# aidagroup/quad-periodic-mpc

Hardware: AMD Instinct MI355X
Metric: QP solves/sec (N=10, 13-state, 12-force) at batch=65536; 1/2/4/8 GPU (higher is better)
Workload: dtype f32

## Files before the change

quad-periodic-mpc_amd/build.py:

```python
from __future__ import annotations

import os
import re
import subprocess
from concurrent.futures import ThreadPoolExecutor

PKG = os.path.dirname(os.path.abspath(__file__))
ROOT = os.path.dirname(PKG)
CSRC = os.path.join(PKG, "csrc")
LIB = os.path.join(PKG, "libcmpc_hip.so")
OBJ = os.path.join(ROOT, "build", "obj")
SOURCES = ["cmpc_tail.hip", "cmpc_wide_w256.hip", "cmpc_wide_w192.hip", "cmpc_class1.hip", "cmpc_wide_w80.hip", "cmpc_wide_w96.hip",
           "cmpc_wide_w120.hip", "cmpc_wide_w128.hip", "cmpc_wide_w144.hip", "cmpc_wide_w80p.hip",
           "cmpc_wide_w96p.hip", "cmpc_wide_w120p.hip", "cmpc_wide_w128p.hip", "cmpc_wide_w80r.hip",
           "cmpc_wide_w96r.hip", "cmpc_wide_w120r.hip", "cmpc_wide_w80pr.hip", "cmpc_wide_w96pr.hip",
           "cmpc_wide_w120pr.hip", "cmpc_wide_w96prd.hip", "cmpc_wide_w120prd.hip", "cmpc_wide_w96rd.hip", "cmpc_wide_w120rd.hip", "cmpc_condense.hip", "cmpc_launch.hip", "cmpc_estimator.hip", "cmpc_assemble.hip",
           "cmpc_admm.hip", "cmpc_quadprog.hip", "cmpc_evaluate.hip", "cmpc_abi.cpp"]
ARCH = os.environ.get("CMPC_OFFLOAD_ARCH", "gfx950")
FLAGS = ["-O3", "-std=c++17", "-fPIC", "-Wall", "-Wno-unused-result", "-fno-slp-vectorize", "-ffp-contract=on"]


def _deps(path: str, seen=None) -> set:
    seen = set() if seen is None else seen
    path = os.path.normpath(path)
    if path in seen or not os.path.exists(path):
        return seen
    seen.add(path)
    for inc in re.findall(r'#include\s+"([^"]+)"', open(path).read()):
        _deps(os.path.join(os.path.dirname(path), inc), seen)
    return seen


def _obj(src: str, defines: tuple) -> str:
    tag = ("_" + "_".join(d.replace("=", "-") for d in defines)) if defines else ""
    return os.path.join(OBJ, f"{src}{tag}.o")


def _stale(target: str, deps) -> bool:
    if not os.path.exists(target):
        return True
    t = os.path.getmtime(target)
    return any(os.path.getmtime(d) > t for d in deps)


def build(force: bool = False, verbose: bool = False, out: str | None = None,
          defines: tuple = ()) -> str:
    lib = out or LIB
    hipcc = os.environ.get("HIPCC", "/opt/rocm/bin/hipcc")
    os.makedirs(OBJ, exist_ok=True)

    def compile_one(src: str) -> str:
        path = os.path.join(CSRC, src)
        obj = _obj(src, defines)
        if not force and not _stale(obj, _deps(path)):
            return obj
        cmd = [hipcc, f"--offload-arch={ARCH}", *FLAGS, *[f"-D{d}" for d in defines], "-c", path,
               "-o", obj + ".tmp"]
        if src.endswith(".cpp"):
            cmd[1:1] = ["-x", "hip"]
        if verbose:
            print(" ".join(cmd), flush=True)
        subprocess.run(cmd, check=True)
        os.replace(obj + ".tmp", obj)
        return obj

    jobs = max(1, min(len(SOURCES), int(os.environ.get("MAX_JOBS", os.cpu_count() or 1))))
    with ThreadPoolExecutor(jobs) as ex:
        objs = list(ex.map(compile_one, SOURCES))
    if not force and not _stale(lib, objs):
        return lib
    tmp = lib + ".tmp"
    subprocess.run([hipcc, f"--offload-arch={ARCH}", "-shared", "-fPIC", "-o", tmp] + objs,
                   check=True)
    os.replace(tmp, lib)
    if out is None:
        build_tools(lib)
        build_multi(lib)
    return lib


MULTI_LIB = os.path.join(PKG, "libcmpc_multi.so")


def build_multi(lib: str = LIB) -> str:
    hipcc = os.environ.get("HIPCC", "/opt/rocm/bin/hipcc")
    src = os.path.join(CSRC, "cmpc_multi.cpp")
    hdrs = [os.path.join(ROOT, "include", h) for h in ("cmpc_multi.h", "cmpc_solver.h")]
    if _stale(MULTI_LIB, [src, lib] + hdrs):
        subprocess.run([hipcc, "-x", "hip", "--offload-arch=" + ARCH, "-O2", "-std=c++17", "-fPIC",
                        "-Wall", "-shared", "-o", MULTI_LIB + ".tmp", src, f"-L{PKG}", "-lcmpc_hip",
                        "-L/opt/rocm/lib", "-lrccl", "-Wl,-rpath,$ORIGIN", f"-Wl,-rpath,{PKG}",
                        "-Wl,-rpath,/opt/rocm/lib"], check=True)
        os.replace(MULTI_LIB + ".tmp", MULTI_LIB)
    exe = os.path.join(PKG, "cmpc_multi_test")
    tsrc = os.path.join(CSRC, "tools", "cmpc_multi_test.cpp")
    if _stale(exe, [tsrc, MULTI_LIB] + hdrs):
        subprocess.run([hipcc, "-x", "hip", "--offload-arch=" + ARCH, "-O2", "-std=c++17", "-o", exe + ".tmp",
                        tsrc, f"-L{PKG}", "-lcmpc_multi", "-lcmpc_hip", "-Wl,-rpath,$ORIGIN",
                        f"-Wl,-rpath,{PKG}"], check=True)
        os.replace(exe + ".tmp", exe)
    exe = os.path.join(PKG, "cmpc_multi_model_test")
    tsrc = os.path.join(CSRC, "tools", "cmpc_multi_model_test.cpp")
    if _stale(exe, [tsrc, MULTI_LIB] + hdrs):
        subprocess.run([hipcc, "-x", "hip", "--offload-arch=" + ARCH, "-O2", "-std=c++17", "-o", exe + ".tmp",
                        tsrc, f"-L{PKG}", "-lcmpc_multi", "-lcmpc_hip", "-Wl,-rpath,$ORIGIN",
                        f"-Wl,-rpath,{PKG}"], check=True)
        os.replace(exe + ".tmp", exe)
    return MULTI_LIB


def build_tools(lib: str = LIB) -> str:
    exe = os.path.join(PKG, "cmpc_abi_latency")
    src = os.path.join(CSRC, "tools", "cmpc_abi_latency.cpp")
    if not _stale(exe, [src, lib]):
        return exe
    subprocess.run(["g++", "-O2", "-std=c++17", "-o", exe + ".tmp", src, f"-L{PKG}", "-lcmpc_hip",
                    f"-Wl,-rpath,$ORIGIN", f"-Wl,-rpath,{PKG}"], check=True)
    os.replace(exe + ".tmp", exe)
    return exe


if __name__ == "__main__":
    import sys
    print(build(force="--force" in sys.argv, verbose=True))
```

quad-periodic-mpc_amd/csrc/cmpc_class1.hip:

```cpp
#include <stdlib.h>

#include "cmpc_common.h"

#ifndef CMPC_W1_WAVES_60
#define CMPC_W1_WAVES_60 4
#endif
#ifndef CMPC_W1_WAVES_PER_EU
#define CMPC_W1_WAVES_PER_EU 4
#endif
#ifndef CMPC_C1_RL
#define CMPC_C1_RL 0
#endif
#ifndef CMPC_TRIP_PRIO_AT
#define CMPC_TRIP_PRIO_AT 0
#endif
#ifndef CMPC_C1_TRIP_PRIO
#define CMPC_C1_TRIP_PRIO 2
#endif
#ifndef C1_PIPE_GRP
#define C1_PIPE_GRP 4
#endif
#ifndef CMPC_C1_CHOL2
#define CMPC_C1_CHOL2 1
#endif
#ifndef CMPC_C1_FUSEDJ
#define CMPC_C1_FUSEDJ 2
#endif
#ifndef CMPC_C1_JPIPE
#define CMPC_C1_JPIPE 1
#endif
#ifndef CMPC_C1_DOT2
#define CMPC_C1_DOT2 0
#endif
#if CMPC_C1_DOT2
#define C1_DOT dot4x2
#else
#define C1_DOT dot4
#endif
#ifndef CMPC_C1_XUNC
#define CMPC_C1_XUNC 1
#endif

#ifdef CMPC_PHASE_PROF
__device__ unsigned long long g_c1_phase[16];
#define C1_MARK(i)                              \
  do {                                          \
    const unsigned long long _n = clock64();    \
    ph[i] += _n - t_last;                       \
    t_last = _n;                                \
  } while (0)
#define C1_SUB(i)                               \
  do {                                          \
    const unsigned long long _n = clock64();    \
    ph[8 + (i)] += _n - t_sub;                  \
    t_sub = _n;                                 \
  } while (0)
#else
#define C1_MARK(i) \
  do {             \
  } while (0)
#define C1_SUB(i) \
  do {            \
  } while (0)
#endif

#ifdef CMPC_PLACE_PROF
constexpr int kPlaceMax = 65536;
__device__ unsigned int g_c1_place[4 * kPlaceMax];
#endif

namespace cmpc {
namespace {

constexpr int NL = 64;

template <int NV>
struct C1Geo {
  static constexpr int NG = NV / 4;
  static constexpr int PSZ = 4 * NG * NV - 8 * NG * (NG - 1);
  __host__ __device__ static constexpr int prow(int r) {
    return 4 * (r >> 2) * NV - 8 * (r >> 2) * ((r >> 2) - 1) + (r & 3) * (NV - 4 * (r >> 2));
  }
  __host__ __device__ static constexpr int prow0(int r) { return prow(r) - (r & ~3); }
  __host__ __device__ static constexpr int tri(int r) { return r * NV - ((r * (r + 1)) >> 1); }
  static_assert(NV * NV - ((NV * (NV + 1)) >> 1) <= 4 * NG * NV - 8 * NG * (NG - 1), "exchange fits P");
};
__device__ __forceinline__ int rcol(int j) { return (j * (j + 1)) >> 1; }
constexpr int rinv_cols(int words) {
  int q = 0;
  while ((q + 1) * (q + 2) <= words) q++;
  return q;
}

constexpr int OFF_E = 0;
constexpr int OFF_ZE = OFF_E + 16 * MAXN;
constexpr int OFF_REC = OFF_ZE + 16 * MAXN;

constexpr int C1_MAXFS = 24;

template <int NV>
struct SharedC1 {
  static_assert(NV % 4 == 0 && NV <= NL, "row width");
  static_assert(NV * (NV + 1) / 2 <= C1Geo<NV>::PSZ, "R must fit in P");
  static_assert(OFF_REC + CMPC_REC_WORDS(MAXN) <= C1Geo<NV>::PSZ, "prep scratch must fit in P");
  static_assert(3 * C1_MAXFS >= NV, "stance list");
  static_assert(NV * (NV + 1) / 2 <= C1Geo<NV>::PSZ - NL, "vbuf in P's tail");
  __device__ __forceinline__ float* vbuf() { return &P[C1Geo<NV>::PSZ - NL]; }
  static constexpr int QI = rinv_cols(C1Geo<NV>::PSZ - NL);
  static constexpr int RB = C1Geo<NV>::PSZ - NL - QI * (QI + 1) / 2;
  static_assert(QI * (QI + 1) / 2 <= RB, "R and R^-1 side by side");
  float P[C1Geo<NV>::PSZ];
  union {
    float BdtT[12][16];
    float ibuf[NL];
    struct {
      float bufA[NL], bufB[NL];
      float cs[2 * NL];
    } gi;
  } u;
  float sub[C1_MAXFS];
  int sfs[C1_MAXFS];
  int blkbase[MAXN + 2];
  unsigned char varblk[NL], varcol[NL];
  unsigned char cmask[NL];
};

__device__ __forceinline__ void lsync() {
  __builtin_amdgcn_wave_barrier();
  asm volatile("" ::: "memory");
}

__device__ __forceinline__ float fdiv(float a, float b) { return a * fast_rcp(b); }

template <int M>
__device__ __forceinline__ void pin(float (&x)[M]) {
#pragma unroll
  for (int c = 0; c < M; c++) asm volatile("" : "+v"(x[c]));
}

template <int LO, int HI, int MA>
__device__ __forceinline__ float pick_col(const float (&x)[MA], int q) {
  static_assert(0 <= LO && LO < HI && HI <= MA, "column range");
  if constexpr (HI - LO == 1) {
    float r = x[LO];
    asm volatile("" : "+v"(r));
    return r;
  } else {
    constexpr int MID = (LO + HI) / 2;
    if (q < MID) return pick_col<LO, MID>(x, q);
    return pick_col<MID, HI>(x, q);
  }
}

#ifndef CMPC_FENCE_COLS
#define CMPC_FENCE_COLS 16
#endif
#define CMPC_SWEEP_FENCE(c)                                                                  \
  do {                                                                                       \
    if (((c) & (CMPC_FENCE_COLS - 1)) == CMPC_FENCE_COLS - 4) __builtin_amdgcn_sched_barrier(0); \
  } while (0)

template <int NV>
__device__ __forceinline__ void solve_c1(const float* __restrict__ rec, const KParams& P,
                                         SharedC1<NV>& sh, float* __restrict__ fout,
                                         uint8_t* __restrict__ st_out, int32_t* __restrict__ it_out,
                                         int* __restrict__ ovf_list, int* __restrict__ ovf_count,
                                         int inst) {
  using G = C1Geo<NV>;
  const int v = threadIdx.x;
  const int N = P.N;
#ifdef CMPC_PHASE_PROF
  unsigned long long ph[16] = {0, 0, 0, 0, 0, 0, 0, 0, 0, 0, 0, 0, 0, 0, 0, 0};
  unsigned long long t_sub = 0;
  unsigned long long t_last = clock64();
#endif
  {
    const float4* src = reinterpret_cast<const float4*>(rec);
    float4* dst = reinterpret_cast<float4*>(&sh.P[OFF_REC]);
    for (int t = v; t < (P.rec_words >> 2); t += 64) dst[t] = src[t];
  }
  lsync();
  const float* srec = &sh.P[OFF_REC];
  const unsigned char* gait = reinterpret_cast<const unsigned char*>(srec + CMPC_REC_HDR + 12 * N);
  int nfs = 0;
  unsigned long long msk0 = 0ull, msk1 = 0ull;
  for (int c0 = 0; c0 < 4 * N; c0 += 64) {
    const int t = c0 + v;
    float ub = 0.f;
    bool f = false;
    if (t < 4 * N) {
      ub = (float)gait[t] * P.f_max;
      f = !(ub < 0.01f && ub > -0.01f);
    }
    const unsigned long long m = __ballot(f);
    if (c0 == 0) msk0 = m; else msk1 = m;
    const int pre = __popcll(m & ((1ull << v) - 1ull));
    if (f && nfs + pre < C1_MAXFS) {
      sh.sfs[nfs + pre] = t;
      sh.sub[nfs + pre] = ub;
    }
    nfs += __popcll(m);
  }
  const int n = 3 * nfs;
  if (n > NV) {
    if (v == 0 && ovf_list) ovf_list[atomicAdd(ovf_count, 1)] = inst;
    return;
  }
  lsync();
  {
    int kb = 0, kc = 0;
    if (v < n) {
      const int fs = sh.sfs[v / 3];
      kb = fs >> 2;
      kc = 3 * (fs & 3) + v % 3;
    }
    sh.varblk[v] = (unsigned char)kb;
    sh.varcol[v] = (unsigned char)kc;
    if (v <= N) {
      const int b0 = 4 * v, b1 = 4 * v - 64;
      const unsigned long long lo = (b0 >= 64) ? msk0 : (msk0 & ((1ull << b0) - 1ull));
      const unsigned long long hi = (b1 <= 0) ? 0ull : (msk1 & ((1ull << b1) - 1ull));
      sh.blkbase[v] = 3 * (__popcll(lo) + __popcll(hi));
    }
    for (int t = v; t < nfs; t += 64) sh.cmask[t] = 0;
  }
  Model md;
  make_model(srec, P.dt, P.mdl, md);
  make_bdt<64>(srec, md, v, sh.u.BdtT);
  CondGeo cg;
  make_cond_geo<true>(srec, md, cg);
  lsync();
  float wts[13];
#pragma unroll
  for (int j = 0; j < 12; j++) wts[j] = P.wts[j];
  wts[12] = 0.f;
  if (v < N) {
    float e[13];
    state_error(srec, md, v, srec + CMPC_REC_HDR + 12 * v, e);
#pragma unroll
    for (int j = 0; j < 13; j++) sh.P[OFF_E + 16 * v + j] = wts[j] * e[j];
  }
  lsync();
  moment_recur(&sh.P[OFF_E], &sh.P[OFF_ZE], N, v);
  lsync();
  C1_MARK(0);

  const bool real = v < n;
  float gv;
  {
    const int kv = real ? sh.varblk[v] : 0;
    const int cv = real ? sh.varcol[v] : 0;
    float b[13], u1[13], u2[13];
#pragma unroll
    for (int j = 0; j < 13; j++) b[j] = real ? sh.u.BdtT[cv][j] : 0.f;
    n1_mul(md, b, u1);
    n1_mul(md, u1, u2);
    gv = grad_from_moments(b, u1, u2, &sh.P[OFF_E + 16 * kv], &sh.P[OFF_ZE + 16 * kv]);
    gv = real ? gv : 0.f;
    lsync();
    const int myrow = G::tri(v);
    float z[13];
#pragma unroll
    for (int j = 0; j < 13; j++) z[j] = 0.f;
    for (int i = N - 1; i >= 0; i--) {
      const bool act = real && (i >= kv);
      const float k = (float)(i - kv);
      const float k2 = 0.5f * k * (k - 1.f);
      float gk[13];
      col_power(b, u1, u2, k, k2, gk);
#pragma unroll
      for (int j = 0; j < 13; j++) gk[j] = act ? gk[j] : 0.f;
      recur(md, wts, gk, z);
      asm volatile("" ::: "memory");
      const int wb = __builtin_amdgcn_readfirstlane(sh.blkbase[i]);
      step_entries(md, cg, sh.u.BdtT, step_mask(msk0, msk1, i), wb, z, [&](int w, float val) {
        if (w == v) val += P.alpha2;
        if (act && w >= v) sh.P[myrow + w] = val;
      });
    }
  }
  lsync();
  C1_MARK(1);

  float slot[NV + 1];
  {
    const int vv = (v < NV) ? v : 0;
    const int myrow = G::tri(vv);
    static_for<0, NV>([&](auto C) {
      constexpr int c = decltype(C)::value;
      const int addr = (c >= vv) ? myrow + c : G::tri(c) + vv;
      const float x = sh.P[addr];
      slot[c] = (real && c < n) ? x : ((c == v) ? 1.f : 0.f);
      if ((c & 7) == 7) __builtin_amdgcn_sched_barrier(0);
    });
    slot[NV] = gv;
  }
  lsync();

  int status = CMPC_OK;
  float my_inv = 1.f;
#if CMPC_C1_CHOL2
  float i0n = 1.f, betan = 0.f, i1n = 1.f, g0n = 0.f, g1n = 0.f;
  auto look = [&](auto JJ) {
    constexpr int j = decltype(JJ)::value, j1 = j + 1;
    constexpr int cj = j & ~3, cj1 = j1 & ~3;
    if constexpr (j1 < NV) {
    float d0 = rl(slot[j], j);
    const float h10 = rl(slot[j], j1);
    if (!(d0 > 0.f)) { status = CMPC_NOT_PD; d0 = 1e-30f; }
    i0n = __builtin_amdgcn_rsqf(d0);
    betan = h10 * (i0n * i0n);
    float d1 = fmaf(-h10, betan, rl(slot[j1], j1));
    if (!(d1 > 0.f)) { status = CMPC_NOT_PD; d1 = 1e-30f; }
    i1n = __builtin_amdgcn_rsqf(d1);
    g0n = rl(slot[NV], j);
    g1n = fmaf(-betan, g0n, rl(slot[NV], j1));
    const float s1 = fmaf(-slot[j], betan, slot[j1]);
#if CMPC_C1_FUSEDJ
    g0n = -g0n * i0n;
    g1n = -g1n * i1n;
    if (v >= cj && v < NV) sh.P[G::prow(j) + v - cj] = (v >= j) ? -slot[j] * i0n : 0.f;
    if (v >= cj1 && v < NV) sh.P[G::prow(j1) + v - cj1] = (v >= j1) ? -s1 * i1n : 0.f;
#else
    if (v >= cj && v < NV) sh.P[G::prow(j) + v - cj] = (v >= j) ? slot[j] : 0.f;
    if (v >= cj1 && v < NV) sh.P[G::prow(j1) + v - cj1] = (v >= j1) ? s1 : 0.f;
#endif
    lsync();
    }
  };
  if (n > 0) look(std::integral_constant<int, 0>{});
  float jc2 = 0.f, jc3 = 0.f;
  (void)jc2; (void)jc3;
  float xunc = 0.f;
  (void)xunc;
  static_for<0, NV / 2>([&](auto KB) {
    constexpr int k = 2 * decltype(KB)::value;
    constexpr int k1 = k + 1, k2 = k + 2;
    constexpr int c0 = k & ~3, c1 = k1 & ~3, c2 = k2 & ~3;
    constexpr int rk = G::prow(k), rk1 = G::prow(k1);
    if (k < n) {
      const float i0 = i0n, beta = betan, i1 = i1n, g0 = g0n, g1 = g1n;
#if CMPC_C1_FUSEDJ
      if (v == k) my_inv = i0;
      if (v == k1) my_inv = i1;
      const float s0 = slot[k];
      const float s1 = fmaf(-s0, beta, slot[k1]);
      const float a0 = (v > k) ? s0 * i0 : 0.f;
      const float a1 = (v > k1) ? s1 * i1 : 0.f;
#else
      if (v == k) { my_inv = i0; sh.u.ibuf[k] = i0; }
      if (v == k1) { my_inv = i1; sh.u.ibuf[k1] = i1; }
      const float s0 = slot[k];
      const float s1 = fmaf(-s0, beta, slot[k1]);
      const float a0 = (v > k) ? -s0 * (i0 * i0) : 0.f;
      const float a1 = (v > k1) ? -s1 * (i1 * i1) : 0.f;
#endif
      slot[NV] = fmaf(a1, g1, fmaf(a0, g0, slot[NV]));
      static_for<c2 / 4, NV / 4>([&](auto JC) {
        constexpr int c = 4 * decltype(JC)::value;
        const float4 r0 = *reinterpret_cast<const float4*>(&sh.P[rk + c - c0]);
        const float4 r1 = *reinterpret_cast<const float4*>(&sh.P[rk1 + c - c1]);
        axpy4(a0, r0, slot[c + 0], slot[c + 1], slot[c + 2], slot[c + 3]);
        axpy4(a1, r1, slot[c + 0], slot[c + 1], slot[c + 2], slot[c + 3]);
        if constexpr (k2 < NV && c == c2) {
          if (k2 < n) look(std::integral_constant<int, k2>{});
        }
        CMPC_SWEEP_FENCE(c);
      });
#if CMPC_C1_FUSEDJ == 2
      if constexpr ((k & 3) == 0) {
        f2v t0 = {(v == k) ? 1.f : 0.f, 0.f}, t1 = {(v == k1) ? 1.f : 0.f, 0.f};
        f2v t2 = {(v == k + 2) ? 1.f : 0.f, 0.f}, t3 = {(v == k + 3) ? 1.f : 0.f, 0.f};
#if CMPC_C1_JPIPE
        piped_sweep<0, k, 1>(
            [&](auto C) {
              constexpr int q = decltype(C)::value;
              return F4x4{*reinterpret_cast<const float4*>(&sh.P[G::prow(q) + k - q]),
                          *reinterpret_cast<const float4*>(&sh.P[G::prow(q + 1) + k - q]),
                          *reinterpret_cast<const float4*>(&sh.P[G::prow(q + 2) + k - q]),
                          *reinterpret_cast<const float4*>(&sh.P[G::prow(q + 3) + k - q])};
            },
            [&](auto C, F4x4 l) {
              constexpr int q = decltype(C)::value;
              const float4 la = l.a, lb = l.b, lc = l.c, ld = l.d;
#else
        static_for<0, k / 4>([&](auto QC) {
          constexpr int q = 4 * decltype(QC)::value;
          const float4 la = *reinterpret_cast<const float4*>(&sh.P[G::prow(q) + k - q]);
          const float4 lb = *reinterpret_cast<const float4*>(&sh.P[G::prow(q + 1) + k - q]);
          const float4 lc = *reinterpret_cast<const float4*>(&sh.P[G::prow(q + 2) + k - q]);
          const float4 ld = *reinterpret_cast<const float4*>(&sh.P[G::prow(q + 3) + k - q]);
#endif
          t0.x = fmaf(slot[q], la.x, t0.x); t1.x = fmaf(slot[q], la.y, t1.x);
          t2.x = fmaf(slot[q], la.z, t2.x); t3.x = fmaf(slot[q], la.w, t3.x);
          t0.y = fmaf(slot[q + 1], lb.x, t0.y); t1.y = fmaf(slot[q + 1], lb.y, t1.y);
          t2.y = fmaf(slot[q + 1], lb.z, t2.y); t3.y = fmaf(slot[q + 1], lb.w, t3.y);
          t0.x = fmaf(slot[q + 2], lc.x, t0.x); t1.x = fmaf(slot[q + 2], lc.y, t1.x);
          t2.x = fmaf(slot[q + 2], lc.z, t2.x); t3.x = fmaf(slot[q + 2], lc.w, t3.x);
          t0.y = fmaf(slot[q + 3], ld.x, t0.y); t1.y = fmaf(slot[q + 3], ld.y, t1.y);
          t2.y = fmaf(slot[q + 3], ld.z, t2.y); t3.y = fmaf(slot[q + 3], ld.w, t3.y);
#if CMPC_C1_JPIPE
            });
#else
          __builtin_amdgcn_sched_barrier(0);
        });
#endif
        const float hk = sh.P[G::prow(k) + k1 - (k & ~3)];
        const float xk = (t0.x + t0.y) * i0;
        slot[k] = xk;
        slot[k1] = fmaf(xk, hk, t1.x + t1.y) * i1;
#if CMPC_C1_XUNC
        xunc = fmaf(slot[k1], g1, fmaf(xk, g0, xunc));
#endif
        jc2 = t2.x + t2.y;
        jc3 = t3.x + t3.y;
        asm volatile("" : "+v"(jc2), "+v"(jc3));
      } else {
        constexpr int km = k - 2;
        const float2 l0 = *reinterpret_cast<const float2*>(&sh.P[G::prow(km) + k - (km & ~3)]);
        const float2 l1 = *reinterpret_cast<const float2*>(&sh.P[G::prow(km + 1) + k - (km & ~3)]);
        const float hk = sh.P[G::prow(k) + k1 - (k & ~3)];
        const float e0 = fmaf(slot[km + 1], l1.x, fmaf(slot[km], l0.x, jc2));
        const float e1 = fmaf(slot[km + 1], l1.y, fmaf(slot[km], l0.y, jc3));
        const float xk = e0 * i0;
        slot[k] = xk;
        slot[k1] = fmaf(xk, hk, e1) * i1;
#if CMPC_C1_XUNC
        xunc = fmaf(slot[k1], g1, fmaf(xk, g0, xunc));
#endif
      }
#elif CMPC_C1_FUSEDJ
      {
        float e0 = (v == k) ? 1.f : 0.f, e1 = (v == k1) ? 1.f : 0.f, o0 = 0.f, o1 = 0.f;
        static_for<0, k>([&](auto JJ) {
          constexpr int j = decltype(JJ)::value;
          const float2 lj = *reinterpret_cast<const float2*>(&sh.P[G::prow(j) + k - (j & ~3)]);
          if constexpr ((j & 1) == 0) {
            e0 = fmaf(slot[j], lj.x, e0);
            e1 = fmaf(slot[j], lj.y, e1);
          } else {
            o0 = fmaf(slot[j], lj.x, o0);
            o1 = fmaf(slot[j], lj.y, o1);
          }
          if constexpr ((j & 7) == 7) __builtin_amdgcn_sched_barrier(0);
        });
        const float hk = sh.P[G::prow(k) + k1 - (k & ~3)];
        const float xk = (e0 + o0) * i0;
        slot[k] = xk;
        slot[k1] = fmaf(xk, hk, e1 + o1) * i1;
      }
#endif
      pin(slot);
    }
  });
#else
  float dnext = 1.f, gnext = 0.f;
  if (n > 0) {
    if (v < NV) sh.P[G::prow(0) + v] = slot[0];
    dnext = rl(slot[0], 0);
    gnext = rl(slot[NV], 0);
    lsync();
  }
  static_for<0, NV>([&](auto KC) {
    constexpr int k = decltype(KC)::value;
    constexpr int c0 = k & ~3;
    constexpr int rk = G::prow(k);
    constexpr int k1 = k + 1;
    constexpr int c1 = k1 & ~3;
    if (k < n) {
      float d = dnext;
      const float gk = gnext;
      if (!(d > 0.f)) { status = CMPC_NOT_PD; d = 1e-30f; }
      const float inv = __builtin_amdgcn_rsqf(d);
      if (v == k) { my_inv = inv; sh.u.ibuf[k] = inv; }
      const float colk = slot[k];
      const float a = (v > k) ? -colk * (inv * inv) : 0.f;
      slot[NV] = fmaf(a, gk, slot[NV]);
      static_for<c0 / 4, NV / 4>([&](auto JC) {
        constexpr int c = 4 * decltype(JC)::value;
        if constexpr (((c / 4) & 3) < CMPC_C1_RL) {
          float s4[4];
          static_for<0, 4>([&](auto EC) {
            constexpr int cc = c + decltype(EC)::value;
            s4[EC] = (cc >= k) ? rl(colk, cc) : 0.f;
          });
          asm volatile("" : "+s"(s4[0]), "+s"(s4[1]), "+s"(s4[2]), "+s"(s4[3]));
          static_for<0, 4>([&](auto EC) {
            constexpr int cc = c + decltype(EC)::value;
            if constexpr (cc >= k) slot[cc] = fmaf(a, s4[EC], slot[cc]);
          });
        } else {
          const float4 r4 = *reinterpret_cast<const float4*>(&sh.P[rk + c - c0]);
          axpy4(a, r4, slot[c + 0], slot[c + 1], slot[c + 2], slot[c + 3]);
        }
        if constexpr (k1 < NV && c == c1) {
          if (k1 < n) {
            constexpr int rk1 = G::prow(k1);
            if (v >= c1 && v < NV) sh.P[rk1 + v - c1] = (v >= k1) ? slot[k1] : 0.f;
            dnext = rl(slot[k1], k1);
            gnext = rl(slot[NV], k1);
            lsync();
          }
        }
        CMPC_SWEEP_FENCE(c);
      });
      pin(slot);
    }
  });
#endif
  const float yv = (v < n) ? slot[NV] * my_inv : 0.f;
  lsync();
  C1_MARK(2);

#if CMPC_C1_CHOL2 && CMPC_C1_FUSEDJ
#else
  static_for<0, NV>([&](auto C) {
    constexpr int c = decltype(C)::value;
    slot[c] = (c == v) ? 1.f : 0.f;
  });
#endif
#if CMPC_C1_CHOL2 && CMPC_C1_FUSEDJ
#elif CMPC_C1_CHOL2
  static_for<0, NV / 2>([&](auto KB) {
    constexpr int k = 2 * decltype(KB)::value;
    constexpr int k1 = k + 1, c2 = (k + 2) & ~3;
    constexpr int c0 = k & ~3, c1 = k1 & ~3;
    constexpr int rk = G::prow(k), rk1 = G::prow(k1);
    if (k < n) {
      const float i0 = sh.u.ibuf[k], i1 = sh.u.ibuf[k1];
      const float h = sh.P[rk + k1 - c0];
      const float x0 = slot[k] * i0;
      const float x1 = fmaf(-h * i0, x0, slot[k1]) * i1;
      const float a0 = -x0 * i0, a1 = -x1 * i1;
#pragma unroll
      for (int c = c2; c < NV; c += 4) {
        const float4 r0 = *reinterpret_cast<const float4*>(&sh.P[rk + c - c0]);
        const float4 r1 = *reinterpret_cast<const float4*>(&sh.P[rk1 + c - c1]);
        axpy4(a0, r0, slot[c + 0], slot[c + 1], slot[c + 2], slot[c + 3]);
        axpy4(a1, r1, slot[c + 0], slot[c + 1], slot[c + 2], slot[c + 3]);
        CMPC_SWEEP_FENCE(c);
      }
      slot[k] = x0;
      slot[k1] = x1;
      pin(slot);
    }
  });
#else
  static_for<0, NV>([&](auto KC) {
    constexpr int k = decltype(KC)::value;
    constexpr int c0 = k & ~3;
    constexpr int rk = G::prow(k);
    if (k < n) {
      const float inv = sh.u.ibuf[k];
      const float xk = slot[k] * inv;
      const float a = -xk * inv;
#pragma unroll
      for (int c = c0; c < NV; c += 4) {
        const float4 r4 = *reinterpret_cast<const float4*>(&sh.P[rk + c - c0]);
        axpy4(a, r4, slot[c + 0], slot[c + 1], slot[c + 2], slot[c + 3]);
        CMPC_SWEEP_FENCE(c);
      }
      slot[k] = xk;
      pin(slot);
    }
  });
#endif

  C1_MARK(3);
#if CMPC_C1_FUSEDJ == 2 && CMPC_C1_XUNC
  (void)yv;
  float xv = (v < n) ? xunc : 0.f;
#else
  sh.vbuf()[v] = yv;
  lsync();
  f2v xacc = {0.f, 0.f};
  piped_sweep<0, NV, C1_PIPE_GRP>(
      [&](auto C) { return *reinterpret_cast<const float4*>(&sh.vbuf()[decltype(C)::value]); },
      [&](auto C, float4 y4) {
        constexpr int c = decltype(C)::value;
        dot4(xacc, slot[c + 0], slot[c + 1], slot[c + 2], slot[c + 3], y4);
      });
  float xv = (v < n) ? -(xacc.x + xacc.y) : 0.f;
  lsync();
#endif

  const float mui = P.mu_inv;
  const float fnorm = rsqrtf(mui * mui + 1.f);
  int q = 0;
  int iters = 0;
  float u_reg = 0.f;
  int act_reg = 0;
  int p = -1;
  Cons cp{};
  float up = 0.f;
  bool rinv_ok = true;
  lsync();
  if (status == CMPC_OK) {
    for (;;) {
      pin(slot);
      const int v = tid_opq();
#ifdef CMPC_PHASE_PROF
      t_sub = clock64();
#endif
      if (p < 0) {
        const float fx = __shfl(xv, 3 * v), fy = __shfl(xv, 3 * v + 1), fz = __shfl(xv, 3 * v + 2);
        float best = 0.f;
        int bid = 0x7fffffff;
        if (v < nfs) {
          const unsigned fm = sh.cmask[v];
          float sl[6];
          sl[0] = (mui * fx + fz) * fnorm;
          sl[1] = (-mui * fx + fz) * fnorm;
          sl[2] = (mui * fy + fz) * fnorm;
          sl[3] = (-mui * fy + fz) * fnorm;
          sl[4] = fz;
          sl[5] = sh.sub[v] - fz;
#pragma unroll
          for (int t = 0; t < 6; t++)
            if (!((fm >> t) & 1u) && sl[t] < best) { best = sl[t]; bid = 6 * v + t; }
        }
        const float xmax = wave_max(fabsf(xv));
        wave_argmin(best, bid);
        const float tol = 1e-5f * fmaxf(1.f, xmax);
        if (bid == 0x7fffffff || best >= -tol) break;
        p = __builtin_amdgcn_readfirstlane(bid);
        cp = decode_cons(p, mui, sh.sub[p / 6]);
        up = 0.f;
      }
      C1_SUB(0);
      if (++iters > P.max_iter + 2 * n) { status = CMPC_MAX_ITER; break; }
#if CMPC_TRIP_PRIO_AT > 0
      if (iters == CMPC_TRIP_PRIO_AT) __builtin_amdgcn_s_setprio(CMPC_C1_TRIP_PRIO);
#endif
      if (v == cp.ia || v == cp.iz) {
        const int boff = (v == cp.iz) ? NL + 16 : 0;
#pragma unroll
        for (int c = 0; c < NV; c++) {
          sh.u.gi.bufA[boff + c] = slot[c];
          if ((c & 15) == 15) __builtin_amdgcn_sched_barrier(0);
        }
      }
      lsync();
      const float dv = (cp.ia != cp.iz) ? fmaf(cp.ca, sh.u.gi.bufA[v], cp.cb * sh.u.gi.bufB[16 + v])
                                        : cp.cb * sh.u.gi.bufB[16 + v];
      const float dm = (v >= q && v < n) ? dv : 0.f;
      sh.vbuf()[v] = dm;
      lsync();
      const float dn = wave_sum((v < n) ? dv * dv : 0.f);
      const float zn = wave_sum(dm * dm);
      f2v zacc = {0.f, 0.f};
      piped_sweep<0, NV, C1_PIPE_GRP>(
          [&](auto C) { return *reinterpret_cast<const float4*>(&sh.vbuf()[decltype(C)::value]); },
          [&](auto C, float4 m4) {
            constexpr int c = decltype(C)::value;
            C1_DOT(zacc, slot[c + 0], slot[c + 1], slot[c + 2], slot[c + 3], m4);
          });
      float zv = zacc.x + zacc.y;
      asm volatile("" : "+v"(zv));
      C1_SUB(1);
      float acc = dv, r_reg = 0.f;
      if (rinv_ok) {
        using S = SharedC1<NV>;
        float a0 = 0.f, a1 = 0.f;
        int j = 0;
        for (; j + 4 <= q; j += 4) {
          const float x0 = sh.P[S::RB + rcol(j) + v], x1 = sh.P[S::RB + rcol(j + 1) + v];
          const float x2 = sh.P[S::RB + rcol(j + 2) + v], x3 = sh.P[S::RB + rcol(j + 3) + v];
          a0 = fmaf((v <= j) ? x0 : 0.f, rl(dv, j), a0);
          a1 = fmaf((v <= j + 1) ? x1 : 0.f, rl(dv, j + 1), a1);
          a0 = fmaf((v <= j + 2) ? x2 : 0.f, rl(dv, j + 2), a0);
          a1 = fmaf((v <= j + 3) ? x3 : 0.f, rl(dv, j + 3), a1);
        }
        for (; j < q; j++) {
          const float x0 = sh.P[S::RB + rcol(j) + v];
          a0 = fmaf((v <= j) ? x0 : 0.f, rl(dv, j), a0);
        }
        r_reg = (v < q) ? a0 + a1 : 0.f;
      } else {
        float pd = 1.f, pv = 0.f;
        if (q > 0) {
          pd = sh.P[rcol(q - 1) + q - 1];
          pv = sh.P[rcol(q - 1) + v];
        }
        for (int i = q - 1; i >= 0; i--) {
          float pd_n = 1.f, pv_n = 0.f;
          if (i > 0) {
            pd_n = sh.P[rcol(i - 1) + i - 1];
            pv_n = sh.P[rcol(i - 1) + v];
          }
          const float ri = fdiv(rl(acc, i), pd);
          if (v < i) acc = fmaf(-pv, ri, acc);
          r_reg = (v == i) ? ri : r_reg;
          pd = pd_n;
          pv = pv_n;
        }
      }
      float t1 = kBigF;
      int kk = 0x7fffffff;
      if (v < q && r_reg > 0.f) { t1 = fmaxf(fdiv(u_reg, r_reg), 0.f); kk = v; }
      wave_argmin(t1, kk);
      const float spv = fmaf(cp.ca, rl(xv, cp.ia), fmaf(cp.cb, rl(xv, cp.iz), -cp.bp));
      const bool zero_step = !(zn > 1e-9f * dn);
      const float t2 = zero_step ? kBigF : -fdiv(spv, zn);
      const float t = fminf(t1, t2);
      if (t >= kBigF) { status = CMPC_INFEASIBLE; break; }
      if (v < q) u_reg = fmaf(-t, r_reg, u_reg);
      up += t;
      if (!zero_step) xv = fmaf(t, zv, xv);
      C1_SUB(2);
      const bool add = !zero_step && t2 <= t1;
      const bool add_u = __builtin_amdgcn_readfirstlane((int)add) != 0;
      float beta = 0.f, sigma = 0.f;
      if (add) {
        const float ts = sqrtf(zn);
        const float dq = rl(dv, q);
        const float sgn = (dq >= 0.f) ? 1.f : -1.f;
        beta = fast_rcp(ts * (ts + fabsf(dq)));
        sigma = sgn * ts;
        sh.vbuf()[v] = (v == q) ? dq + sgn * ts : dm;
        const int offq = rcol(q);
        if (v < q) sh.P[offq + v] = dv;
        if (v == q) {
          sh.P[offq + q] = -sgn * ts;
          u_reg = up;
          act_reg = p;
        }
        if (rinv_ok) {
          if (q < SharedC1<NV>::QI) {
            const float irho = 1.f / (-sgn * ts);
            const int offi = SharedC1<NV>::RB + rcol(q);
            if (v < q) sh.P[offi + v] = -r_reg * irho;
            if (v == q) sh.P[offi + q] = irho;
          } else {
            rinv_ok = false;
          }
        }
        if (v == 0) sh.cmask[p / 6] |= (unsigned char)(1u << (p % 6));
      } else {
        sh.vbuf()[v] = 0.f;
        const int k = __builtin_amdgcn_readfirstlane(kk);
        const int ak = rli(act_reg, k);
        if (v == 0) sh.cmask[ak / 6] &= (unsigned char)~(1u << (ak % 6));
        const int a_nx = lane_next_i(act_reg, act_reg);
        const float u_nx = lane_next(u_reg, u_reg);
        if (v >= k && v < q - 1) { act_reg = a_nx; u_reg = u_nx; }
        if (v < k || v > q - 2) *reinterpret_cast<float2*>(&sh.u.gi.cs[2 * v]) = make_float2(1.f, 0.f);
        const bool in_c = v >= k && v <= q - 2;
        float top = in_c ? sh.P[rcol(v + 1) + k] : 0.f;
        lsync();
        for (int r = 0; r < k; r++) {
          const float x = in_c ? sh.P[rcol(v + 1) + r] : 0.f;
          lsync();
          if (in_c) sh.P[rcol(v) + r] = x;
          lsync();
        }
        for (int j = k; j <= q - 2; j++) {
          const bool on = in_c && v >= j;
          const float bot = on ? sh.P[rcol(v + 1) + j + 1] : 0.f;
          lsync();
          const float a0 = rl(top, j), b0 = rl(bot, j);
          const float h = sqrtf(a0 * a0 + b0 * b0);
          float cc = 1.f, sn = 0.f;
          if (h > 0.f) { const float ih = fast_rcp(h); cc = a0 * ih; sn = b0 * ih; }
          if (on) {
            sh.P[rcol(v) + j] = fmaf(cc, top, sn * bot);
            top = fmaf(-sn, top, cc * bot);
          }
          if (v == 0) *reinterpret_cast<float2*>(&sh.u.gi.cs[2 * j]) = make_float2(cc, sn);
          lsync();
        }
        if (rinv_ok) {
          using S = SharedC1<NV>;
          const int i = v;
          const bool live = i < q && i != k;
          const int i2 = (i > k) ? i - 1 : i;
          int j = (i > k) ? i - 1 : k;
          float carry = (live && j >= i) ? sh.P[S::RB + rcol(j) + i] : 0.f;
          for (int jj = k; jj <= q - 2; jj++) {
            const float2 cs2 = *reinterpret_cast<const float2*>(&sh.u.gi.cs[2 * jj]);
            const float b = (live && jj >= j && jj + 1 >= i) ? sh.P[S::RB + rcol(jj + 1) + i] : 0.f;
            lsync();
            if (live && jj >= j) {
              sh.P[S::RB + rcol(jj) + i2] = fmaf(cs2.x, carry, cs2.y * b);
              carry = fmaf(-cs2.y, carry, cs2.x * b);
            }
          }
        }
      }
      lsync();
      C1_SUB(3);
      {
        const int qs = __builtin_amdgcn_readfirstlane(q);
        const float bt = -beta * fmaf(sigma, pick_col<0, NV>(slot, qs), zv);
        piped_sweep<0, NV, C1_PIPE_GRP>(
            [&](auto C) { return *reinterpret_cast<const float4*>(&sh.vbuf()[decltype(C)::value]); },
            [&](auto C, float4 w4) {
              constexpr int c = decltype(C)::value;
              axpy4(bt, w4, slot[c + 0], slot[c + 1], slot[c + 2], slot[c + 3]);
            });
      }
      C1_SUB(4);
      if (!add_u) {
        static_for<0, NV - 1>([&](auto JC) {
          constexpr int j = decltype(JC)::value;
          const float2 cs2 = *reinterpret_cast<const float2*>(&sh.u.gi.cs[2 * j]);
          const float x0 = slot[j], x1 = slot[j + 1];
          slot[j] = fmaf(cs2.x, x0, cs2.y * x1);
          slot[j + 1] = fmaf(-cs2.y, x0, cs2.x * x1);
          if ((j & 7) == 7) __builtin_amdgcn_sched_barrier(0);
        });
      }
      C1_SUB(5);
#ifdef CMPC_PHASE_PROF
      ph[14] += add ? 0ull : 1ull;
#endif
      if (add) {
        q++;
        p = -1;
      } else {
        q--;
      }
      lsync();
    }
  }

  C1_MARK(4);
  const bool ok = (status == CMPC_OK);
  for (int t = v; t < 12 * N; t += 64) sh.P[t] = 0.f;
  lsync();
  if (ok && v < n) sh.P[12 * sh.varblk[v] + sh.varcol[v]] = xv;
  lsync();
  for (int t = 4 * v; t < P.out_cols; t += 256)
    *reinterpret_cast<float4*>(&fout[t]) = *reinterpret_cast<const float4*>(&sh.P[t]);
  if (v == 0) {
    st_out[0] = (uint8_t)status;
    if (it_out) it_out[0] = iters;
  }
#ifdef CMPC_PHASE_PROF
  C1_MARK(5);
  if (v == 0) {
    ph[6] = 1;
    ph[7] = (unsigned long long)iters;
#pragma unroll
    for (int i = 0; i < 16; i++) atomicAdd(&g_c1_phase[i], ph[i]);
  }
#endif
}

}

template <int NV>
__global__ __launch_bounds__(64, NV == 60 ? CMPC_W1_WAVES_60 : CMPC_W1_WAVES_PER_EU) void cmpc_solve_c1_kernel(
    const float* __restrict__ recs, int batch, KParams P, float* __restrict__ forces,
    uint8_t* __restrict__ status, int32_t* __restrict__ iters, const int* __restrict__ in_list,
    const int* __restrict__ in_count, int* __restrict__ ovf_list, int* __restrict__ ovf_count) {
  __shared__ SharedC1<NV> sh;
  int t = blockIdx.x;
  if (in_list) {
    if (t >= *in_count) return;
    t = in_list[t];
  } else if (t >= batch) {
    return;
  }
#ifdef CMPC_PLACE_PROF
  const unsigned long long t_start = wall_clock64();
  const unsigned hw_id = __builtin_amdgcn_s_getreg((31 << 11) | 4);
  const unsigned xcc_id = __builtin_amdgcn_s_getreg((31 << 11) | 20);
#endif
  solve_c1<NV>(recs + (size_t)t * P.rec_words, P, sh, forces + (size_t)t * P.out_cols, status + t,
               iters ? iters + t : nullptr, ovf_list, ovf_count, t);
#ifdef CMPC_PLACE_PROF
  const unsigned long long t_end = wall_clock64();
  if (threadIdx.x == 0 && t < kPlaceMax) {
    g_c1_place[4 * t + 0] = hw_id;
    g_c1_place[4 * t + 1] = xcc_id;
    g_c1_place[4 * t + 2] = (unsigned)t_start;
    g_c1_place[4 * t + 3] = (unsigned)t_end;
  }
#endif
}

hipError_t launch_class1(int nv, const float* d_recs, int batch, const KParams& P, float* d_forces,
                         uint8_t* d_status, int32_t* d_iters, const int* in_list, const int* in_count,
                         int* ovf_list, int* ovf_count, int grid, hipStream_t stream) {
  if (grid <= 0) return hipSuccess;
  static const unsigned dyn = (unsigned)diag_knob("CMPC_C1_DYN_LDS", 0);
  if (nv == 60)
    hipLaunchKernelGGL(cmpc_solve_c1_kernel<60>, dim3(grid), dim3(64), dyn, stream, d_recs, batch, P,
                       d_forces, d_status, d_iters, in_list, in_count, ovf_list, ovf_count);
  else
    hipLaunchKernelGGL(cmpc_solve_c1_kernel<64>, dim3(grid), dim3(64), dyn, stream, d_recs, batch, P,
                       d_forces, d_status, d_iters, in_list, in_count, ovf_list, ovf_count);
  return hipGetLastError();
}

}

#ifdef CMPC_PHASE_PROF
extern "C" int cmpc_debug_phase_read(unsigned long long* out) {
  if (hipMemcpyFromSymbol(out, HIP_SYMBOL(g_c1_phase), sizeof(unsigned long long) * 16) != hipSuccess)
    return -1;
  unsigned long long z[16] = {0, 0, 0, 0, 0, 0, 0, 0, 0, 0, 0, 0, 0, 0, 0, 0};
  return hipMemcpyToSymbol(HIP_SYMBOL(g_c1_phase), z, sizeof(z)) == hipSuccess ? 0 : -1;
}
#endif

#ifdef CMPC_PLACE_PROF
extern "C" int cmpc_debug_place_read(unsigned int* out, int n) {
  if (n > kPlaceMax) n = kPlaceMax;
  return hipMemcpyFromSymbol(out, HIP_SYMBOL(g_c1_place), sizeof(unsigned int) * 4 * n) == hipSuccess ? 0 : -1;
}
#endif
```

Before: 50.96 million.

## Use 4x4x1 MFMA broadcasts for rank-1 updates in class1 Cholesky and Householder sweeps

Replaces the shared-memory broadcast plus per-lane axpy rank-1 updates in the pair-step Cholesky and the Householder reflector application with v_mfma_f32_4x4x1f32. The instruction's broadcast block selector lets each lane's register value serve as the broadcast column, so the vbuf round trip and several wave barriers are removed. An optional level (3) also moves the fused-J dot products onto MFMA. This adds matrix-core latency and constrains register allocation, and it depends on the MFMA lane and block semantics being correct for the wave layout. A standalone MFMA probe tool is added to the build.

```diff
diff --git a/quad-periodic-mpc_amd/build.py b/quad-periodic-mpc_amd/build.py
--- a/quad-periodic-mpc_amd/build.py
+++ b/quad-periodic-mpc_amd/build.py
@@ -112,11 +112,22 @@
 def build_tools(lib: str = LIB) -> str:
     exe = os.path.join(PKG, "cmpc_abi_latency")
     src = os.path.join(CSRC, "tools", "cmpc_abi_latency.cpp")
-    if not _stale(exe, [src, lib]):
-        return exe
-    subprocess.run(["g++", "-O2", "-std=c++17", "-o", exe + ".tmp", src, f"-L{PKG}", "-lcmpc_hip",
-                    f"-Wl,-rpath,$ORIGIN", f"-Wl,-rpath,{PKG}"], check=True)
-    os.replace(exe + ".tmp", exe)
+    if _stale(exe, [src, lib]):
+        subprocess.run(["g++", "-O2", "-std=c++17", "-o", exe + ".tmp", src, f"-L{PKG}", "-lcmpc_hip",
+                        f"-Wl,-rpath,$ORIGIN", f"-Wl,-rpath,{PKG}"], check=True)
+        os.replace(exe + ".tmp", exe)
+    build_mfma_probe()
+    return exe
+
+
+def build_mfma_probe() -> str:
+    hipcc = os.environ.get("HIPCC", "/opt/rocm/bin/hipcc")
+    exe = os.path.join(PKG, "cmpc_mfma_probe")
+    src = os.path.join(CSRC, "tools", "cmpc_mfma_probe.cpp")
+    if _stale(exe, [src]):
+        subprocess.run([hipcc, "-x", "hip", "--offload-arch=" + ARCH, "-O2", "-std=c++17", "-o",
+                        exe + ".tmp", src], check=True)
+        os.replace(exe + ".tmp", exe)
     return exe
 
 
diff --git a/quad-periodic-mpc_amd/csrc/cmpc_class1.hip b/quad-periodic-mpc_amd/csrc/cmpc_class1.hip
--- a/quad-periodic-mpc_amd/csrc/cmpc_class1.hip
+++ b/quad-periodic-mpc_amd/csrc/cmpc_class1.hip
@@ -39,6 +39,12 @@
 #endif
 #ifndef CMPC_C1_XUNC
 #define CMPC_C1_XUNC 1
+#endif
+#ifndef CMPC_C1_MFMA
+#define CMPC_C1_MFMA 2
+#endif
+#if CMPC_C1_MFMA && !(CMPC_C1_CHOL2 && CMPC_C1_FUSEDJ)
+#error "CMPC_C1_MFMA needs the pair-step Cholesky with the fused J (CMPC_C1_CHOL2, CMPC_C1_FUSEDJ)"
 #endif
 
 #ifdef CMPC_PHASE_PROF
@@ -131,6 +137,21 @@
 }
 
 __device__ __forceinline__ float fdiv(float a, float b) { return a * fast_rcp(b); }
+
+#if CMPC_C1_MFMA
+typedef float f4m __attribute__((ext_vector_type(4)));
+template <int C>
+__device__ __forceinline__ void mfma_chunk(float col, float coef, float& x0, float& x1, float& x2,
+                                           float& x3) {
+  static_assert((C & 3) == 0 && C >= 0 && C < 64, "chunk start");
+  f4m acc = {x0, x1, x2, x3};
+  acc = __builtin_amdgcn_mfma_f32_4x4x1f32(col, coef, acc, 4, C / 4, 0);
+  x0 = acc[0];
+  x1 = acc[1];
+  x2 = acc[2];
+  x3 = acc[3];
+}
+#endif
 
 template <int M>
 __device__ __forceinline__ void pin(float (&x)[M]) {
@@ -301,6 +322,9 @@
   float my_inv = 1.f;
 #if CMPC_C1_CHOL2
   float i0n = 1.f, betan = 0.f, i1n = 1.f, g0n = 0.f, g1n = 0.f;
+#if CMPC_C1_MFMA
+  float pub0n = 0.f, pub1n = 0.f;
+#endif
   auto look = [&](auto JJ) {
     constexpr int j = decltype(JJ)::value, j1 = j + 1;
     constexpr int cj = j & ~3, cj1 = j1 & ~3;
@@ -319,13 +343,22 @@
 #if CMPC_C1_FUSEDJ
     g0n = -g0n * i0n;
     g1n = -g1n * i1n;
+#if CMPC_C1_MFMA
+    pub0n = (v >= j) ? -slot[j] * i0n : 0.f;
+    pub1n = (v >= j1) ? -s1 * i1n : 0.f;
+    if (v >= cj && v < NV) sh.P[G::prow(j) + v - cj] = pub0n;
+    if (v >= cj1 && v < NV) sh.P[G::prow(j1) + v - cj1] = pub1n;
+#else
     if (v >= cj && v < NV) sh.P[G::prow(j) + v - cj] = (v >= j) ? -slot[j] * i0n : 0.f;
     if (v >= cj1 && v < NV) sh.P[G::prow(j1) + v - cj1] = (v >= j1) ? -s1 * i1n : 0.f;
+#endif
 #else
     if (v >= cj && v < NV) sh.P[G::prow(j) + v - cj] = (v >= j) ? slot[j] : 0.f;
     if (v >= cj1 && v < NV) sh.P[G::prow(j1) + v - cj1] = (v >= j1) ? s1 : 0.f;
 #endif
+#if !CMPC_C1_MFMA
     lsync();
+#endif
     }
   };
   if (n > 0) look(std::integral_constant<int, 0>{});
@@ -356,6 +389,25 @@
       const float a1 = (v > k1) ? -s1 * (i1 * i1) : 0.f;
 #endif
       slot[NV] = fmaf(a1, g1, fmaf(a0, g0, slot[NV]));
+#if CMPC_C1_MFMA
+      if constexpr (c2 < NV) {
+        const float p0 = pub0n, p1 = pub1n;
+        mfma_chunk<c2>(p0, a0, slot[c2 + 0], slot[c2 + 1], slot[c2 + 2], slot[c2 + 3]);
+        mfma_chunk<c2>(p1, a1, slot[c2 + 0], slot[c2 + 1], slot[c2 + 2], slot[c2 + 3]);
+        if constexpr (k2 < NV) {
+          if (k2 < n) look(std::integral_constant<int, k2>{});
+        }
+        static_for<c2 / 4 + 1, NV / 4>([&](auto JC) {
+          constexpr int c = 4 * decltype(JC)::value;
+          mfma_chunk<c>(p0, a0, slot[c + 0], slot[c + 1], slot[c + 2], slot[c + 3]);
+        });
+        static_for<c2 / 4 + 1, NV / 4>([&](auto JC) {
+          constexpr int c = 4 * decltype(JC)::value;
+          mfma_chunk<c>(p1, a1, slot[c + 0], slot[c + 1], slot[c + 2], slot[c + 3]);
+        });
+      }
+      lsync();
+#else
       static_for<c2 / 4, NV / 4>([&](auto JC) {
         constexpr int c = 4 * decltype(JC)::value;
         const float4 r0 = *reinterpret_cast<const float4*>(&sh.P[rk + c - c0]);
@@ -367,10 +419,34 @@
         }
         CMPC_SWEEP_FENCE(c);
       });
+#endif
 #if CMPC_C1_FUSEDJ == 2
       if constexpr ((k & 3) == 0) {
         f2v t0 = {(v == k) ? 1.f : 0.f, 0.f}, t1 = {(v == k1) ? 1.f : 0.f, 0.f};
         f2v t2 = {(v == k + 2) ? 1.f : 0.f, 0.f}, t3 = {(v == k + 3) ? 1.f : 0.f, 0.f};
+#if CMPC_C1_MFMA >= 3
+        {
+          f4m te = {t0.x, t1.x, t2.x, t3.x}, to = {0.f, 0.f, 0.f, 0.f};
+          const int vc = (v < NV) ? v : NV - 1;
+          piped_sweep<0, k, 2>(
+              [&](auto C) {
+                constexpr int q = decltype(C)::value;
+                return float4{sh.P[G::prow0(q) + vc], sh.P[G::prow0(q + 1) + vc],
+                              sh.P[G::prow0(q + 2) + vc], sh.P[G::prow0(q + 3) + vc]};
+              },
+              [&](auto C, float4 l) {
+                constexpr int q = decltype(C)::value;
+                te = __builtin_amdgcn_mfma_f32_4x4x1f32(l.x, slot[q], te, 4, k / 4, 0);
+                to = __builtin_amdgcn_mfma_f32_4x4x1f32(l.y, slot[q + 1], to, 4, k / 4, 0);
+                te = __builtin_amdgcn_mfma_f32_4x4x1f32(l.z, slot[q + 2], te, 4, k / 4, 0);
+                to = __builtin_amdgcn_mfma_f32_4x4x1f32(l.w, slot[q + 3], to, 4, k / 4, 0);
+              });
+          t0 = {te[0], to[0]};
+          t1 = {te[1], to[1]};
+          t2 = {te[2], to[2]};
+          t3 = {te[3], to[3]};
+        }
+#else
 #if CMPC_C1_JPIPE
         piped_sweep<0, k, 1>(
             [&](auto C) {
@@ -404,6 +480,7 @@
 #else
           __builtin_amdgcn_sched_barrier(0);
         });
+#endif
 #endif
         const float hk = sh.P[G::prow(k) + k1 - (k & ~3)];
         const float xk = (t0.x + t0.y) * i0;
@@ -711,13 +788,20 @@
       const bool add = !zero_step && t2 <= t1;
       const bool add_u = __builtin_amdgcn_readfirstlane((int)add) != 0;
       float beta = 0.f, sigma = 0.f;
+#if CMPC_C1_MFMA >= 2
+      float wreg = 0.f;
+#endif
       if (add) {
         const float ts = sqrtf(zn);
         const float dq = rl(dv, q);
         const float sgn = (dq >= 0.f) ? 1.f : -1.f;
         beta = fast_rcp(ts * (ts + fabsf(dq)));
         sigma = sgn * ts;
+#if CMPC_C1_MFMA >= 2
+        wreg = (v == q) ? dq + sgn * ts : dm;
+#else
         sh.vbuf()[v] = (v == q) ? dq + sgn * ts : dm;
+#endif
         const int offq = rcol(q);
         if (v < q) sh.P[offq + v] = dv;
         if (v == q) {
@@ -737,7 +821,9 @@
         }
         if (v == 0) sh.cmask[p / 6] |= (unsigned char)(1u << (p % 6));
       } else {
+#if CMPC_C1_MFMA < 2
         sh.vbuf()[v] = 0.f;
+#endif
         const int k = __builtin_amdgcn_readfirstlane(kk);
         const int ak = rli(act_reg, k);
         if (v == 0) sh.cmask[ak / 6] &= (unsigned char)~(1u << (ak % 6));
@@ -792,12 +878,19 @@
       {
         const int qs = __builtin_amdgcn_readfirstlane(q);
         const float bt = -beta * fmaf(sigma, pick_col<0, NV>(slot, qs), zv);
+#if CMPC_C1_MFMA >= 2
+        static_for<0, NV / 4>([&](auto JC) {
+          constexpr int c = 4 * decltype(JC)::value;
+          mfma_chunk<c>(wreg, bt, slot[c + 0], slot[c + 1], slot[c + 2], slot[c + 3]);
+        });
+#else
         piped_sweep<0, NV, C1_PIPE_GRP>(
             [&](auto C) { return *reinterpret_cast<const float4*>(&sh.vbuf()[decltype(C)::value]); },
             [&](auto C, float4 w4) {
               constexpr int c = decltype(C)::value;
               axpy4(bt, w4, slot[c + 0], slot[c + 1], slot[c + 2], slot[c + 3]);
             });
+#endif
       }
       C1_SUB(4);
       if (!add_u) {
```

Measured after the change: 52.58 million (median of 6 runs). 3.2% higher.
